# zhengjingsen/LidarDetection

Measured on AMD Instinct MI355X. Metric: frames/sec (fwd+NMS) PointPillar-KITTI, higher is better.
Workload: dtype f32; 1 GPU; PointPillar-KITTI bs=16 per GPU, fp32, eval BN folded: HIP voxelize + PFN; dense 2D backbone = first layer from the pillars (sparse implicit GEMM), stride-1 3x3 layers as Winograd F(4x4,3x3) on the fp32 MFMA, strided deblocks as one fused MFMA GEMM (all this repo's HIP), the two stride-2 3x3 layers MIOpen, stride-1 deblock + 1x1 heads hipBLASLt; exact HIP top-k + decode + batched rotated NMS; clou; replicas=1

## Files before the change

### include/lidar_hip.h

```cpp
#ifndef LIDAR_HIP_H
#define LIDAR_HIP_H

#include <stddef.h>
#include <stdint.h>

#ifdef __cplusplus
extern "C" {
#endif

#define LIDAR_OK 0
#define LIDAR_ERR_ARG (-1)
#define LIDAR_ERR_LAUNCH (-2)
#define LIDAR_ERR_WORKSPACE (-3)
#define LIDAR_ERR_UNSUPPORTED (-4)

size_t lidar_voxelize_workspace_bytes(int batch, int n_max, int max_voxels);
int lidar_voxelize_workspace_init(void *ws, size_t ws_bytes, int batch, int n_max, int max_voxels, void *stream);
int lidar_voxelize(const float *points, const int *point_offsets, int batch, int n_max, int num_features,
                   const float *range6, const float *voxel_size3, const int *grid3, int max_points,
                   int max_voxels, int compact, int algo, float *voxels, int *coords, int *num_points,
                   int *voxel_offsets, void *ws, size_t ws_bytes, void *stream);
int lidar_voxelize_hostoff(const float *points, const int *point_offsets, const int *host_offsets, int batch, int n_max,
                           int num_features, const float *range6, const float *voxel_size3, const int *grid3, int max_points,
                           int max_voxels, int compact, int algo, float *voxels, int *coords, int *num_points,
// ... 238 lines not shown
                            void *ws, size_t ws_bytes, void *stream);

size_t lidar_deconv_packed_floats(int K, int N);
int lidar_deconv_supported(int K, int s, int C_up);
int lidar_deconv_pack_weights(const float *W, int K, int N, float *packed, void *stream);
int lidar_deconv_gemm_nhwc(const float *in, int B, int h, int w, int K, const float *packed, const float *bias, int relu, int s, int C_up,
                           float *out, int out_C, int out_off, void *stream);

#define LIDAR_DECONV_TRAIN_MIN_K 16
#define LIDAR_DECONV_TRAIN_MIN_CUP 32
#define LIDAR_DECONV_TRAIN_MAX_C 512
int lidar_deconv_train_supported(int K, int s, int C_up);
size_t lidar_deconv_wgrad_workspace_bytes(int B, int h, int w, int K, int s, int C_up);
int lidar_deconv_dgrad_nhwc(const float *g, int g_ld, const float *W, int B, int h, int w, int K, int s, int C_up, float *dx, int dx_ld,
                            void *stream);
int lidar_deconv_wgrad_nhwc(const float *x, int x_ld, const float *g, int g_ld, int B, int h, int w, int K, int s, int C_up, float *dw,
                            void *ws, size_t ws_bytes, void *stream);

int lidar_anchor_scores(const float *head, long long n_loc, int row_stride, int cls_off, int anchors_per_loc, int num_class,
                        float score_thresh, float *scores, unsigned char *labels, void *stream);
int lidar_decode_topk(const float *head, int batch, long long locs_per_frame, int row_stride, int box_off, int dir_off,
                      int anchors_per_loc, int num_dir_bins, const long long *top_idx, int k, const float *anchors,
                      float dir_offset, float dir_limit_offset, float period, float *boxes, void *stream);
size_t lidar_topk_workspace_bytes(int batch, long long n);
int lidar_topk_workspace_init(void *ws, size_t ws_bytes, int batch, long long n, void *stream);
int lidar_anchor_scores_hist(const float *head, int batch, long long locs_per_frame, int row_stride, int cls_off, int anchors_per_loc,
                             int num_class, float score_thresh, float *scores, unsigned char *labels, void *ws, size_t ws_bytes,
                             void *stream);
int lidar_topk_desc(const float *scores, int batch, long long n, int k, float valid_min, float score_max, int hist_ready,
                    float *top_scores, long long *top_idx, int *counts, void *ws, size_t ws_bytes, void *stream);
int lidar_post_nms_gather(const float *boxes, const float *top_scores, const long long *top_idx, const unsigned char *labels,
                          const long long *keep, const int *num_keep, int batch, int k, long long n, int keep_stride, int post,
                          float *out_boxes, float *out_scores, long long *out_labels, int *out_num, void *stream);

size_t lidar_anchor_assign_workspace_bytes(int batch, int max_gt, int num_classes);
int lidar_anchor_assign(const float *const *anchors, const long long *counts, const long long *per_loc, const long long *out_off,
                        const float *matched, const float *unmatched, const int *remap, int num_classes, int anchor_dim,
                        long long a_total, const signed char *class_of_id, const float *gt, const float *gt_enlarged, int batch,
                        int max_gt, int gt_cols, int code_size, int sincos, int norm_by_num_examples, int *labels, float *targets,
                        float *weights, void *ws, size_t ws_bytes, void *stream);

int lidar_atss_assign_supported(const long long *counts, int num_sets, int anchor_dim, int gt_cols, int code_size, int sincos,
                                int topk, int max_gt, int match_height);
size_t lidar_atss_assign_workspace_bytes(int batch, int max_gt, int num_sets, int topk);
int lidar_atss_assign(const float *const *anchors, const long long *counts, int num_sets, int anchor_dim, const float *gt, int batch,
                      int max_gt, int gt_cols, int code_size, int sincos, int topk, int match_height, int *labels, float *targets,
// ... 126 lines not shown
```

### lidardetection_amd/_lib.py

```python
import ctypes as C
import os

_HERE = os.path.dirname(os.path.abspath(__file__))
SO_PATH = os.environ.get("LIDAR_HIP_SO") or os.path.join(_HERE, "csrc", "liblidar_hip.so")

vp, i32, f32, sz = C.c_void_p, C.c_int, C.c_float, C.c_size_t

SIGNATURES = {
    "lidar_voxelize_workspace_bytes": (sz, [i32, i32, i32]),
    "lidar_voxelize_workspace_init": (i32, [vp, sz, i32, i32, i32, vp]),
    "lidar_voxelize": (i32, [vp, vp, i32, i32, i32, vp, vp, vp, i32, i32, i32, i32, vp, vp, vp, vp, vp, sz, vp]),
    "lidar_voxelize_hostoff": (i32, [vp, vp, vp, i32, i32, i32, vp, vp, vp, i32, i32, i32, i32, vp, vp, vp, vp, vp, sz, vp]),
    "lidar_voxelize_error_flag": (i32, [vp, sz, i32, i32, i32]),
    "lidar_timer_create": (vp, []),
    "lidar_timer_destroy": (None, [vp]),
    "lidar_voxelize_time_next": (None, [vp]),
    "lidar_timer_elapsed_ms": (C.c_float, [vp]),
    "lidar_timer_parts_ms": (i32, [vp, vp]),
    "lidar_voxelize_set_error_mirror": (i32, [vp, sz, i32, i32, i32, vp, vp]),
    "lidar_pillar_vfe": (i32, [vp, vp, vp, i32, vp, i32, i32, vp, vp, vp, i32, vp, vp, i32, i32, i32, vp, vp]),
    "lidar_mean_vfe": (i32, [vp, vp, i32, i32, i32, i32, vp, vp]),
    "lidar_pillar_scatter_workspace_bytes": (sz, [i32, i32, i32]),
    "lidar_pillar_scatter": (i32, [vp, vp, i32, i32, vp, i32, i32, i32, i32, i32, vp, vp, sz, vp]),
    "lidar_pillar_scatter_update": (i32, [vp, vp, i32, i32, vp, i32, i32, i32, i32, vp, vp, vp, vp]),
# ... 97 lines not shown
    "lidar_wino43_pack_weights": (i32, [vp, i32, i32, vp, vp]),
    "lidar_wino43_conv3x3_nhwc": (i32, [vp, i32, i32, i32, i32, i32, vp, vp, i32, i32, vp, i32, i32, vp]),
    "lidar_wino43s_packed_floats": (sz, [i32, i32]),
    "lidar_wino43s_supported": (i32, [i32, i32]),
    "lidar_wino43s_pack_weights": (i32, [vp, i32, i32, vp, vp]),
    "lidar_wino43s_conv3x3_nhwc": (i32, [vp, i32, i32, i32, i32, i32, vp, vp, i32, i32, vp, i32, i32, vp]),
    "lidar_wino43_wgrad_supported": (i32, [i32, i32]),
    "lidar_wino43_wgrad_workspace_bytes": (sz, [i32, i32, i32, i32, i32]),
    "lidar_wino43_wgrad_nhwc": (i32, [vp, i32, vp, i32, i32, i32, i32, i32, i32, vp, vp, sz, vp]),
    "lidar_wino_conv3x3_grouped_nhwc": (i32, [vp, i32, i32, i32, i32, i32, i32, vp, vp, i32, vp, i32, i32, vp]),
    "lidar_wino_conv3x3_grouped_compact_nhwc": (i32, [vp, i32, i32, i32, i32, i32, i32, vp, vp, i32, vp, vp, vp, i32, i32, vp]),
    "lidar_deconv_packed_floats": (sz, [i32, i32]),
    "lidar_deconv_supported": (i32, [i32, i32, i32]),
    "lidar_deconv_pack_weights": (i32, [vp, i32, i32, vp, vp]),
    "lidar_deconv_gemm_nhwc": (i32, [vp, i32, i32, i32, i32, vp, vp, i32, i32, i32, vp, i32, i32, vp]),
    "lidar_deconv_train_supported": (i32, [i32, i32, i32]),
    "lidar_deconv_wgrad_workspace_bytes": (sz, [i32, i32, i32, i32, i32, i32]),
    "lidar_deconv_dgrad_nhwc": (i32, [vp, i32, vp, i32, i32, i32, i32, i32, i32, vp, i32, vp]),
    "lidar_deconv_wgrad_nhwc": (i32, [vp, i32, vp, i32, i32, i32, i32, i32, i32, i32, vp, vp, sz, vp]),
    "lidar_anchor_scores": (i32, [vp, C.c_longlong, i32, i32, i32, i32, f32, vp, vp, vp]),
    "lidar_decode_topk": (i32, [vp, i32, C.c_longlong, i32, i32, i32, i32, i32, vp, i32, vp, f32, f32, f32, vp, vp]),
    "lidar_topk_workspace_bytes": (sz, [i32, C.c_longlong]),
    "lidar_topk_workspace_init": (i32, [vp, sz, i32, C.c_longlong, vp]),
    "lidar_anchor_scores_hist": (i32, [vp, i32, C.c_longlong, i32, i32, i32, i32, f32, vp, vp, vp, sz, vp]),
    "lidar_topk_desc": (i32, [vp, i32, C.c_longlong, i32, f32, f32, i32, vp, vp, vp, vp, sz, vp]),
    "lidar_post_nms_gather": (i32, [vp, vp, vp, vp, vp, vp, i32, i32, C.c_longlong, i32, i32, vp, vp, vp, vp, vp]),
    "lidar_anchor_assign_workspace_bytes": (sz, [i32, i32, i32]),
    "lidar_anchor_assign": (i32, [vp, vp, vp, vp, vp, vp, vp, i32, i32, C.c_longlong, vp, vp, vp, i32, i32, i32, i32, i32, i32, vp,
                                  vp, vp, vp, sz, vp]),
    "lidar_atss_assign_supported": (i32, [vp, i32, i32, i32, i32, i32, i32, i32, i32]),
    "lidar_atss_assign_workspace_bytes": (sz, [i32, i32, i32, i32]),
    "lidar_atss_assign": (i32, [vp, vp, i32, i32, vp, i32, i32, i32, i32, i32, i32, i32, vp, vp, vp, vp, sz, vp]),
    "lidar_proposal_target_supported": (i32, [i32, i32, i32, i32]),
    "lidar_proposal_target": (i32, [vp, vp, vp, vp, vp, i32, i32, i32, i32, i32, i32, vp, i32, i32, f32, f32, f32, f32, f32, vp, vp,
                                    vp, vp, vp, vp, vp, vp, vp, vp, vp, vp, vp, vp, vp]),
    "lidar_augment_supported": (i32, [i32, i32, i32, i32]),
    "lidar_augment_workspace_bytes": (sz, [i32, i32, i32, i32]),
    "lidar_augment": (i32, [vp, vp, i32, i32, vp, vp, i32, i32, vp, vp, vp, vp, i32, i32, vp, i32, i32, vp, vp, vp, vp, vp, vp, vp,
                            vp, vp, vp, i32, i32, C.c_longlong, i32, vp, vp, vp, vp, vp, vp, sz, vp]),
    "lidar_anchor_loss_workspace_bytes": (sz, [i32, vp, i32]),
    "lidar_anchor_loss_forward": (i32, [vp, vp, vp, vp, vp, vp, i32, vp, vp, vp, i32, i32, C.c_longlong, i32, i32, i32, vp, vp, i32,
                                        vp, vp, sz, vp]),
    "lidar_anchor_loss_backward": (i32, [vp, vp, vp, vp, vp, vp, i32, vp, vp, vp, i32, i32, C.c_longlong, i32, i32, i32, vp, vp, i32,
                                         vp, vp, vp, vp, vp, sz, vp]),
    "lidar_roi_loss_supported": (i32, [i32, i32, i32, i32, i32, i32]),
    "lidar_roi_loss_workspace_bytes": (sz, [i32, i32]),
# ... 138 lines not shown
```

### lidardetection_amd/anchor_post.py

```python
import numpy as np
import torch

from . import _lib


_TOPK_WS = {}


def topk_supported(n, k, valid_min=None, hist=False):
    return n % 4 == 0 and 0 < k <= 4096 and n < 2 ** 31 and (not hist or valid_min is None or float(valid_min) > 0.0)


def drop_topk_workspace(ws):
    for key in [k for k, v in _TOPK_WS.items() if v is ws]:
        del _TOPK_WS[key]


def topk_workspace(batch, n, device):
    key = (str(device), int(batch), int(n), int(_lib.stream().value or 0))
    ws = _TOPK_WS.get(key)
    if ws is None:
        L = _lib.lib()
        nbytes = L.lidar_topk_workspace_bytes(batch, n)
        ws = torch.empty(nbytes, dtype=torch.uint8, device=device)
# ... 34 lines not shown
    _lib.check(_lib.lib().lidar_anchor_scores(_lib.ptr(head), n_loc, C, int(cls_off), int(anchors_per_loc), int(num_class),
                                              float(score_thresh), _lib.ptr(scores), _lib.ptr(labels), _lib.stream()),
               "lidar_anchor_scores")
    return scores, labels


def decode_topk(head, top_idx, anchors, anchors_per_loc, box_off, dir_off, num_dir_bins, dir_offset, dir_limit_offset):
    _lib.require_cuda(head, top_idx, anchors, allow=(torch.int64,))
    _lib.require_last(anchors, 7, "anchors")
    if top_idx.dtype != torch.int64:
        raise _lib.LidarHipError("decode_topk: top_idx must be int64 (torch.topk indices)")
    B, C = head.shape[0], head.shape[-1]
    locs = head.numel() // C // B
    k = top_idx.shape[1]
    boxes = torch.empty((B, k, 7), dtype=torch.float32, device=head.device)
    period = float(np.float32(2 * np.pi / num_dir_bins)) if num_dir_bins else 1.0
    _lib.check(_lib.lib().lidar_decode_topk(_lib.ptr(head), B, locs, C, int(box_off), int(dir_off), int(anchors_per_loc),
                                            int(num_dir_bins), _lib.ptr(top_idx), k, _lib.ptr(anchors), float(np.float32(dir_offset)),
                                            float(np.float32(dir_limit_offset)), period, _lib.ptr(boxes), _lib.stream()),
               "lidar_decode_topk")
    return boxes


def post_nms_gather(boxes, top_scores, top_idx, labels_all, keep, num_keep, post):
    _lib.require_cuda(boxes, top_scores, top_idx, labels_all, keep, num_keep, allow=(torch.int64, torch.uint8))
    if (boxes.dtype != torch.float32 or top_scores.dtype != torch.float32 or top_idx.dtype != torch.int64 or labels_all.dtype != torch.uint8
            or keep.dtype != torch.int64 or num_keep.dtype != torch.int32):
        raise _lib.LidarHipError("post_nms_gather: boxes / scores f32, top_idx / keep int64, labels uint8, num_keep int32")
    _lib.require_last(boxes, 7, "boxes")
    B, k = top_scores.shape
    n = labels_all.shape[1]
    post = int(post)
    dev = boxes.device
    out_boxes = torch.empty((B, post, 7), dtype=torch.float32, device=dev)
    out_scores = torch.empty((B, post), dtype=torch.float32, device=dev)
    out_labels = torch.empty((B, post), dtype=torch.int64, device=dev)
    out_num = torch.empty((B,), dtype=torch.int32, device=dev)
    _lib.check(_lib.lib().lidar_post_nms_gather(_lib.ptr(boxes), _lib.ptr(top_scores), _lib.ptr(top_idx), _lib.ptr(labels_all), _lib.ptr(keep),
                                                _lib.ptr(num_keep), B, k, n, keep.shape[1], post, _lib.ptr(out_boxes), _lib.ptr(out_scores),
                                                _lib.ptr(out_labels), _lib.ptr(out_num), _lib.stream()), "lidar_post_nms_gather")
    return out_boxes, out_scores, out_labels, out_num
```

### lidardetection_amd/bev_backbone.py

```python
import ctypes as C
import os
from typing import NamedTuple, Optional

import torch
import torch.nn as nn
import torch.nn.functional as F

from . import _lib, wino, workspace


def bias_act_(x, bias, relu=True, out=None, out_offset=0):
    _lib.require_cuda(bias)
    if not (x.is_cuda and x.dim() == 4 and x.is_contiguous(memory_format=torch.channels_last)):
        raise _lib.LidarHipError("bias_act_: expected a channels-last CUDA tensor")
    B, C, H, W = x.shape
    out, out_offset = (x, 0) if out is None else _lib.nhwc_out("bias_act_", B, (H, W), C, x.device, out, out_offset)
    _lib.check(_lib.lib().lidar_bias_act_nhwc(_lib.ptr(x), _lib.ptr(bias), B * H * W, C, int(bool(relu)), _lib.ptr(out),
                                              out.shape[1], int(out_offset), _lib.stream()), "lidar_bias_act_nhwc")
    return out


_LT_GEMM = [os.environ.get("LIDAR_BEV_LT_GEMM", "1") != "0"]
_SPLIT_MIN = [int(os.environ.get("LIDAR_BEV_SPLIT_MIN", "8"))]
_SPLIT = [int(os.environ.get("LIDAR_BEV_SPLIT", "2"))]
_WINO = [os.environ.get("LIDAR_BEV_WINO", "1") != "0"]
_DECONV = [os.environ.get("LIDAR_BEV_DECONV", "1") != "0"]
_SPARSE_FIRST = [os.environ.get("LIDAR_BEV_SPARSE_FIRST", "1") != "0"]


def _lt_gemm(a_ptr, M, K, w_kn, bias, relu, d_ptr, ldd, device):
    ws = workspace.get("dense_gemm", 32 << 20, device)
    st = _lib.lib().lidar_dense_gemm_bias_act(a_ptr, M, K, _lib.ptr(w_kn), w_kn.shape[1], _lib.ptr(bias), int(bool(relu)), d_ptr, ldd,
                                              _lib.ptr(ws), ws.numel(), _lib.stream())
    if st == -4:
        return False
    _lib.check(st, "lidar_dense_gemm_bias_act")
    return True


def _side_streams(device, n):
    from .spconv import conv as _sc, modules as _sm
    dev = torch.device(device)
    out = []
    for pool in (_sc._SIDE_STREAMS, _sm._RULEBOOK_STREAMS)[:n]:
        st = pool.get(dev)
        if st is None:
            st = pool[dev] = torch.cuda.Stream(dev, priority=-1)
        out.append(st)
    return out

# ... 181 lines not shown
                w, b = _fold(up.weight, bn, 1, up.bias)
                s = up.stride[0]
                if tuple(up.kernel_size) == tuple(up.stride) and s == up.stride[1] and \
                        tuple(up.padding) == (0, 0) and tuple(up.output_padding) == (0, 0):
                    w_kn = w.permute(0, 2, 3, 1).reshape(w.shape[0], -1).contiguous()
                    upc = FoldedDeblock("gemm", w_kn, None, b, s, ())
                    if _DECONV[0] and w.is_cuda and s > 1 and deconv_supported(w_kn.shape[0], s, b.numel()):
                        upc = upc._replace(kind="deconv_mfma", packed=deconv_pack(w_kn))
                else:
                    upc = FoldedDeblock("deconv", w.contiguous(memory_format=torch.channels_last), None, b, 0,
                                        (up.stride, up.padding, up.output_padding))
            else:
                w, b = _fold(up.weight, bn, 0, up.bias)
                upc = FoldedDeblock("conv", w.contiguous(memory_format=torch.channels_last), None, b, 0, (up.stride, up.padding))
            self.stages.append((convs, upc))
        self.up_channels = [up.shift.numel() for _, up in self.stages]
        for h in heads:
            assert tuple(h.kernel_size) == (1, 1) and tuple(h.stride) == (1, 1)
        self.head_split = [h.weight.shape[0] for h in heads]
        if heads:
            self.head_wt = torch.cat([h.weight.detach().flatten(1) for h in heads], 0).t().contiguous()
            self.head_b = torch.cat([h.bias.detach() if h.bias is not None else h.weight.new_zeros(h.weight.shape[0])
                                     for h in heads], 0).contiguous()
        self._cats = {}
        self._streams = None
        self._first_sparse = None
        c0 = self.stages[0][0][0]
        w0, b0, st0, pad0 = c0.weight, c0.shift, c0.stride, c0.pad
        k0 = w0.shape[2]
        if (w0.is_cuda and w0.shape[2] == w0.shape[3] and st0[0] == st0[1] and pad0[0] == pad0[1] and k0 * k0 <= 31
                and c0.dilation == (1, 1) and c0.groups == 1 and c0.zero_pad is None):
            from .spconv import ops as _sops
            if _sops.sorted_gemm_supported(k0 * k0, w0.shape[1], w0.shape[0]):
                self._first_sparse = (w0.permute(2, 3, 1, 0).reshape(k0 * k0, w0.shape[1], w0.shape[0]).contiguous(), b0, k0, int(st0[0]), int(pad0[0]))

    def first_layer_from_pillars(self, pm):
        from . import pillar_ops
        from .spconv import ops as _sops
        w9, b0, k0, st0, pad0 = self._first_sparse
        nbr, OH, OW = pillar_ops.pillar_conv_table(pm.coords, pm.B, pm.nx, pm.ny, k0, st0, pad0, pm.num_voxels_dev)
        order = _sops.mask_order(nbr)
        out = _sops.indice_conv_fused(pm.features, nbr, w9, b0, None, True, order)
        return out.view(pm.B, OH, OW, w9.shape[2]).permute(0, 3, 1, 2)

    def sparse_first_ok(self):
        return self._first_sparse is not None and _SPARSE_FIRST[0]

# ... 1 lines not shown
        x, cat, off = canvas, None, 0
        for si, (convs, up) in enumerate(self.stages):
            for ci, cv in enumerate(convs):
                if first_done and si == 0 and ci == 0:
                    continue
                if cv.wino is not None and _WINO[0] and x.is_contiguous(memory_format=torch.channels_last):
                    x = wino.conv3x3_auto(x, cv.wino, cv.weight.shape[0], cv.shift, True)
                    continue
                if cv.zero_pad is not None:
                    x = F.pad(x, cv.zero_pad)
                x = _cl(F.conv2d(x, cv.weight, None, cv.stride, cv.pad, cv.dilation, cv.groups))
                bias_act_(x, cv.shift)
            B, _, h, w = x.shape
            y = None
            if up.kind in ("deconv", "conv"):
                y = _cl((F.conv_transpose2d if up.kind == "deconv" else F.conv2d)(x, up.weight, None, *up.args))
            oh, ow = (h * up.stride, w * up.stride) if y is None else y.shape[2:]
            if cat is None:
                shape = (B, sum(self.up_channels), oh, ow)
                cat = self._cats.get(slot)
                if cat is None or cat.shape != shape or cat.device != x.device:
                    cat = self._cats[slot] = torch.empty(shape, dtype=torch.float32, device=x.device,
                                                         memory_format=torch.channels_last)
            if y is not None:
                bias_act_(y, up.shift, out=cat, out_offset=off)
            else:
                self._deblock_gemm(x, up, cat, off)
            off += up.shift.numel()
        return cat

    def _deblock_gemm(self, x, up, cat, off):
        B, K, h, w = x.shape
        if up.kind == "deconv_mfma" and deconv_fits(B, K, h, w, up.stride, cat.shape[1]):
            return deconv_gemm_into_(x, up.packed, up.shift, up.stride, cat, off)
        if up.kind == "gemm" and up.stride == 1 and _LT_GEMM[0]:
            if gemm_bias_act_into_(x, up.weight, up.shift, cat, off):
                return cat
            _LT_GEMM[0] = False
        y = rows_gemm(x.permute(0, 2, 3, 1).reshape(B * h * w, -1), up.weight)
        return bias_act_upsample_(y, up.shift, B, h, w, up.stride, cat, off)

    def stale(self):
        return params_key(self.sources) != self.source_key

    def merged(self, canvas):
        first_done = False
        if not torch.is_tensor(canvas):
            if self.sparse_first_ok():
                canvas, first_done = self.first_layer_from_pillars(canvas), True
            else:
                canvas = canvas.dense()
        B = canvas.shape[0]
        if 1 < _SPLIT[0] <= 2 and canvas.is_cuda and B % _SPLIT[0] == 0 and B // _SPLIT[0] >= _SPLIT_MIN[0]:
            return self._merged_split(canvas, _SPLIT[0], first_done)
        cat = self.features(canvas, first_done=first_done)
        B, C, H, W = cat.shape
        out = rows_gemm(cat.permute(0, 2, 3, 1).reshape(B * H * W, C), self.head_wt, self.head_b)
        return out.view(B, H, W, -1)

    def _merged_split(self, canvas, n, first_done=False):
        dev = canvas.device
        cur = torch.cuda.current_stream(dev)
        self._streams = _side_streams(dev, n)
        B, hb = canvas.shape[0], canvas.shape[0] // n
        out = None
        for i, st in enumerate(self._streams):
            st.wait_stream(cur)
            with torch.cuda.stream(st):
                cat = self.features(canvas[i * hb:(i + 1) * hb], slot=i + 1, first_done=first_done)
                _, C, H, W = cat.shape
                if out is None:
                    with torch.cuda.stream(cur):
                        out = torch.empty((B, H, W, self.head_wt.shape[1]), dtype=torch.float32, device=dev)
                    st.wait_stream(cur)
                out.record_stream(st)
                rows_gemm(cat.permute(0, 2, 3, 1).reshape(hb * H * W, C), self.head_wt, self.head_b, out=out[i * hb:(i + 1) * hb].view(hb * H * W, -1))
        for st in self._streams:
            cur.wait_stream(st)
        return out

    def __call__(self, canvas):
        return torch.split(self.merged(canvas), self.head_split, dim=-1)
```

### lidardetection_amd/csrc/anchor_post.hip

```cpp
#include "common.h"

__device__ __forceinline__ float sigmoid_ref(float x) { return 1.0f / (1.0f + expf(-x)); }

__global__ __launch_bounds__(256) void anchor_scores_kernel(const float *__restrict__ head, long long n_anchor, int row_stride,
                                                            int cls_off, int A, int ncls, float thresh,
                                                            float *__restrict__ scores, unsigned char *__restrict__ labels) {
    const long long i = (long long)blockIdx.x * 256 + threadIdx.x;
    if (i >= n_anchor) return;
    const long long loc = i / A;
    const int a = (int)(i - loc * A);
    const float *p = head + loc * row_stride + cls_off + a * ncls;
    float best = sigmoid_ref(p[0]);
    int bl = 0;
    for (int c = 1; c < ncls; ++c) {
        const float s = sigmoid_ref(p[c]);
        if (s > best) { best = s; bl = c; }
    }
    scores[i] = (best >= thresh) ? best : -1.0f;
    labels[i] = (unsigned char)bl;
}

__global__ __launch_bounds__(256) void decode_topk_kernel(const float *__restrict__ head, int batch, long long locs_per_frame,
                                                          int row_stride, int box_off, int dir_off, int A, int nbins,
                                                          const long long *__restrict__ top_idx, int k,
                                                          const float *__restrict__ anchors, float dir_offset,
                                                          float dir_limit_offset, float period, float *__restrict__ boxes) {
    const long long j = (long long)blockIdx.x * 256 + threadIdx.x;
    if (j >= (long long)batch * k) return;
    const int b = (int)(j / k);
    const long long idx = top_idx[j];
    const long long loc = idx / A;
    const int a = (int)(idx - loc * A);
    const float *row = head + ((long long)b * locs_per_frame + loc) * row_stride;
    const float *t = row + box_off + a * 7;
    const float *an = anchors + idx * 7;
    const float xa = an[0], ya = an[1], za = an[2], dxa = an[3], dya = an[4], dza = an[5], ra = an[6];
    const float diagonal = sqrtf(dxa * dxa + dya * dya);
    float *o = boxes + j * 7;
    o[0] = t[0] * diagonal + xa;
    o[1] = t[1] * diagonal + ya;
    o[2] = t[2] * dza + za;
    o[3] = expf(t[3]) * dxa;
    o[4] = expf(t[4]) * dya;
    o[5] = expf(t[5]) * dza;
    float rg = t[6] + ra;
    if (nbins > 0) {
        const float *d = row + dir_off + a * nbins;
        int lab = 0;
        float bestd = d[0];
        for (int c = 1; c < nbins; ++c)
            if (d[c] > bestd) { bestd = d[c]; lab = c; }
        const float inv_period = 1.0f / period;
        const float val = rg - dir_offset;
        const float fl = floorf(val * inv_period + dir_limit_offset);
        const float dir_rot = val - fl * period;
        rg = dir_rot + dir_offset + period * (float)lab;
    }
    o[6] = rg;
}

LIDAR_EXPORT int lidar_anchor_scores(const float *head, long long n_loc, int row_stride, int cls_off, int anchors_per_loc,
                                     int num_class, float score_thresh, float *scores, unsigned char *labels, void *stream) {
    if (n_loc < 0 || anchors_per_loc <= 0 || num_class <= 0 || cls_off < 0 ||
        cls_off + anchors_per_loc * num_class > row_stride)
        return LIDAR_ERR_ARG;
    if (n_loc == 0) return LIDAR_OK;
    if (!head || !scores || !labels) return LIDAR_ERR_ARG;
    const long long n = n_loc * anchors_per_loc;
    const long long blocks = (n + 255) / 256;
    if (blocks > 0x7fffffffll) return LIDAR_ERR_ARG;
    hipLaunchKernelGGL(anchor_scores_kernel, dim3((unsigned)blocks), dim3(256), 0, (hipStream_t)stream, head, n, row_stride, cls_off,
                       anchors_per_loc, num_class, score_thresh, scores, labels);
    return lidar_check_launch("lidar_anchor_scores");
}

LIDAR_EXPORT int lidar_decode_topk(const float *head, int batch, long long locs_per_frame, int row_stride, int box_off,
                                   int dir_off, int anchors_per_loc, int num_dir_bins, const long long *top_idx, int k,
                                   const float *anchors, float dir_offset, float dir_limit_offset, float period, float *boxes,
                                   void *stream) {
    if (batch < 0 || k < 0 || locs_per_frame < 0 || anchors_per_loc <= 0 || box_off < 0 ||
        box_off + anchors_per_loc * 7 > row_stride || num_dir_bins < 0 ||
        (num_dir_bins > 0 && (dir_off < 0 || dir_off + anchors_per_loc * num_dir_bins > row_stride)))
        return LIDAR_ERR_ARG;
    if (batch == 0 || k == 0) return LIDAR_OK;
    if (!head || !top_idx || !anchors || !boxes) return LIDAR_ERR_ARG;
    const long long n = (long long)batch * k;
    hipLaunchKernelGGL(decode_topk_kernel, dim3((unsigned)((n + 255) / 256)), dim3(256), 0, (hipStream_t)stream, head, batch,
                       locs_per_frame, row_stride, box_off, dir_off, anchors_per_loc, num_dir_bins, top_idx, k, anchors, dir_offset,
                       dir_limit_offset, period, boxes);
    return lidar_check_launch("lidar_decode_topk");
}

__global__ __launch_bounds__(256) void post_nms_gather_kernel(const float *__restrict__ boxes, const float *__restrict__ top_scores,
                                                              const long long *__restrict__ top_idx, const unsigned char *__restrict__ labels,
                                                              const long long *__restrict__ keep, const int *__restrict__ num_keep,
                                                              int batch, int k, long long n, int keep_stride, int post,
                                                              float *__restrict__ out_boxes, float *__restrict__ out_scores,
                                                              long long *__restrict__ out_labels, int *__restrict__ out_num) {
    const int j = blockIdx.x * 256 + threadIdx.x;
    if (j >= batch * post) return;
    const int b = j / post, s = j - b * post;
    const int nk = min(num_keep[b], post);
    if (s == 0) out_num[b] = nk;
    long long c = 0;
    if (s < nk) c = min(max(keep[(size_t)b * keep_stride + s], 0ll), (long long)k - 1);
    const float *src = boxes + ((size_t)b * k + c) * 7;
    float *dst = out_boxes + (size_t)j * 7;
#pragma unroll
    for (int q = 0; q < 7; ++q) dst[q] = src[q];
    out_scores[j] = top_scores[(size_t)b * k + c];
    const long long a = min(max(top_idx[(size_t)b * k + c], 0ll), n - 1);
    out_labels[j] = (long long)labels[(size_t)b * n + a] + 1;
}
// ... 14 lines not shown
```

### lidardetection_amd/pointpillar.py

```python
import numpy as np
import torch
import torch.nn as nn

from . import anchor_loss, anchor_post, pillar_ops, synth
from .bev_backbone import FoldedBEVBackbone, collect_params, params_key
from .bev_train import TrainBEVBackbone, _check_deblock, _check_wgrad
from .ext import iou3d_nms_cuda
from .voxelizer import BatchVoxelizer, grid_size_of

KITTI_ANCHORS = [
    ([3.9, 1.6, 1.56], [0, 1.57], -1.78),
    ([0.8, 0.6, 1.73], [0, 1.57], -0.6),
    ([1.76, 0.6, 1.73], [0, 1.57], -0.6),
]


def make_bev_backbone(cin=64, layer_nums=(3, 5, 5), strides=(2, 2, 2), filters=(64, 128, 256),
                      up_strides=(1, 2, 4), up_filters=(128, 128, 128)):
    blocks, deblocks = nn.ModuleList(), nn.ModuleList()
    c_in = [cin, *filters[:-1]]
    for i in range(len(layer_nums)):
        layers = [nn.ZeroPad2d(1), nn.Conv2d(c_in[i], filters[i], 3, stride=strides[i], padding=0, bias=False),
                  nn.BatchNorm2d(filters[i], eps=1e-3, momentum=0.01), nn.ReLU()]
        for _ in range(layer_nums[i]):
# ... 96 lines not shown
        if self._bev is None or self._bev.stale():
            self._bev = FoldedBEVBackbone(self.blocks, self.deblocks, [self.conv_cls, self.conv_box, self.conv_dir_cls])
        return self._bev

    def voxelize(self, points, point_offsets, host_offsets=None, timer=None):
        return self.voxelizer(points, point_offsets, self.n_max, compact=True, out=self._vox_out, resident=self.resident_voxels,
                              host_offsets=host_offsets, timer=timer)

    def vfe_scatter(self, vox):
        w, s, t = self._pfn_folded()
        total = vox["voxel_offsets"][self.B:self.B + 1]
        feat = pillar_ops.pillar_vfe(vox["voxels"], vox["voxel_num_points"], vox["voxel_coords"], w, s, t,
                                     self.voxel_size, self.pc_range, num_voxels_dev=total)
        if self.channels_last:
            def dense(f, c, n):
                if self._canvas is None:
                    self._canvas = pillar_ops.ResidentCanvas(self.B, f.shape[1], self.ny, self.nx, vox["voxels"].shape[0], f.device)
                return self._canvas.update(f, c, num_voxels_dev=n)
            if self.fold_bn and self._bev_folded().sparse_first_ok():
                return pillar_ops.PillarMap(feat, vox["voxel_coords"], total, self.B, self.nx, self.ny, dense)
            return dense(feat, vox["voxel_coords"], total)
        return pillar_ops.pillar_scatter(feat, vox["voxel_coords"], self.B, self.nx, self.ny, num_voxels_dev=total)

    def backbone_head(self, canvas):
        if self.fold_bn:
            return (self._bev_folded().merged(canvas),)
        return self.backbone_head_stock(canvas if torch.is_tensor(canvas) else canvas.dense())

    def split_heads(self, head):
        a = self.num_anchor_per_loc
        cls, box, dirs = torch.split(head, [a * self.num_class, a * 7, a * self.num_dir_bins], dim=-1)
        return (cls.reshape(self.B, -1, self.num_class), box.reshape(self.B, -1, 7), dirs.reshape(self.B, -1, self.num_dir_bins))

    def backbone_head_stock(self, canvas):
        ups, x = [], canvas
        for blk, de in zip(self.blocks, self.deblocks):
            x = blk(x)
            ups.append(de(x))
        return self._head_maps(torch.cat(ups, dim=1))

    def _head_maps(self, x):
        cls = self.conv_cls(x).permute(0, 2, 3, 1).reshape(self.B, -1, self.num_class)
        box = self.conv_box(x).permute(0, 2, 3, 1).reshape(self.B, -1, 7)
        dirs = self.conv_dir_cls(x).permute(0, 2, 3, 1).reshape(self.B, -1, self.num_dir_bins)
        return cls, box, dirs

    def backbone_head_train(self, canvas, wgrad="library", deblock="library"):
        _check_wgrad(wgrad, "PointPillarKITTI.backbone_head_train")
        _check_deblock(deblock, "PointPillarKITTI.backbone_head_train")
        if not self.channels_last:
            raise pillar_ops._lib.LidarHipError("PointPillarKITTI.backbone_head_train needs the channels-last model (channels_last=True)")
        key = ("_bev_train" if wgrad == "library" else "_bev_train_" + wgrad) + ("" if deblock == "library" else "_" + deblock)
        if self.__dict__.get(key) is None:
# ... 54 lines not shown
        diag = torch.sqrt(dxa ** 2 + dya ** 2)
        boxes = torch.cat([xt * diag + xa, yt * diag + ya, zt * dza + za, torch.exp(dxt) * dxa, torch.exp(dyt) * dya,
                           torch.exp(dzt) * dza, rt + ra], dim=-1)
        period = 2 * np.pi / self.num_dir_bins
        dir_labels = torch.max(dir_logits, dim=-1)[1]
        rot = limit_period(boxes[..., 6] - self.dir_offset, self.dir_limit_offset, period)
        boxes[..., 6] = rot + self.dir_offset + period * dir_labels.to(boxes.dtype)
        return boxes

    def post_process(self, *heads):
        if len(heads) == 1:
            return self.post_process_fused(heads[0])
        return self.post_process_torch(*heads)

    def select_topk(self, masked, k):
        if masked.is_cuda and anchor_post.topk_supported(masked.shape[1], k, self.score_thresh):
            return anchor_post.topk_desc(masked, k, self.score_thresh)[:2]
        return torch.topk(masked, k, dim=1)

    def post_process_fused(self, head):
        a = self.num_anchor_per_loc
        n = head.shape[1] * head.shape[2] * a if head.dim() == 4 else head.shape[1] * a
        k = min(self.nms_pre, n)
        if anchor_post.topk_supported(n, k, self.score_thresh, hist=True):
            ws = anchor_post.topk_workspace(head.shape[0], n, head.device)
            try:
                masked, labels_all = anchor_post.anchor_scores(head, a, self.num_class, self.score_thresh, cls_off=0, topk_ws=ws)
                top_scores, top_idx, counts = anchor_post.topk_desc(masked, k, self.score_thresh, ws, hist_ready=True)
            except BaseException:
                anchor_post.drop_topk_workspace(ws)
                raise
        else:
            masked, labels_all = anchor_post.anchor_scores(head, a, self.num_class, self.score_thresh, cls_off=0)
            top_scores, top_idx = torch.topk(masked, k, dim=1)
            counts = (top_scores >= self.score_thresh).sum(dim=1).to(torch.int32)
        boxes = anchor_post.decode_topk(head, top_idx, self.anchors, a, box_off=a * self.num_class,
                                        dir_off=a * (self.num_class + 7), num_dir_bins=self.num_dir_bins,
                                        dir_offset=self.dir_offset, dir_limit_offset=self.dir_limit_offset)
        post = min(self.nms_post, k)
        keep, num = iou3d_nms_cuda.nms_batch(boxes, counts, self.nms_thresh, max_keep=post)
        return anchor_post.post_nms_gather(boxes, top_scores, top_idx, labels_all, keep, num, post)

    def post_process_torch(self, cls, box, dirs):
        scores_all, labels_all = torch.sigmoid(cls).max(dim=-1)
        masked = torch.where(scores_all >= self.score_thresh, scores_all, scores_all.new_full((), -1.0))
        k = min(self.nms_pre, masked.shape[1])
        top_scores, top_idx = torch.topk(masked, k, dim=1)
        counts = (top_scores >= self.score_thresh).sum(dim=1).to(torch.int32)
        gi = top_idx.unsqueeze(-1)
        boxes = self.decode(torch.gather(box, 1, gi.expand(-1, -1, 7)), self.anchors[top_idx],
                            torch.gather(dirs, 1, gi.expand(-1, -1, self.num_dir_bins))).contiguous()
        return self._nms_and_gather(boxes, top_scores, top_idx, labels_all, counts, k)

    def _nms_and_gather(self, boxes, top_scores, top_idx, labels_all, counts, k):
        post = min(self.nms_post, k)
        keep, num = iou3d_nms_cuda.nms_batch(boxes, counts, self.nms_thresh, max_keep=post)
        sel = keep[:, :post].clamp_(0, k - 1)
        num = torch.clamp(num, max=post)
        valid = torch.arange(post, device=sel.device).unsqueeze(0) < num.unsqueeze(1)
        sel = torch.where(valid, sel, torch.zeros_like(sel))
        out_boxes = torch.gather(boxes, 1, sel.unsqueeze(-1).expand(-1, -1, 7))
# ... 10 lines not shown
```

Baseline: 3284 frames/s.

## Defer box/direction head GEMM to top-k rows only

The dense 1x1 head GEMM now computes only the class columns over every BEV location. The box and direction logits are computed later by a new HIP kernel, and only for the top-k selected anchors, reading the backbone concat buffers directly. A matching decode kernel consumes those compact rows. This cuts most of the head GEMM's FLOPs and output bandwidth. The cost is a gather-style per-row dot-product kernel, plus a staleness hazard if the concat buffers are overwritten before post-processing.

```diff
diff --git a/include/lidar_hip.h b/include/lidar_hip.h
--- a/include/lidar_hip.h
+++ b/include/lidar_hip.h
@@ -284,6 +284,13 @@
 int lidar_decode_topk(const float *head, int batch, long long locs_per_frame, int row_stride, int box_off, int dir_off,
                       int anchors_per_loc, int num_dir_bins, const long long *top_idx, int k, const float *anchors,
                       float dir_offset, float dir_limit_offset, float period, float *boxes, void *stream);
+#define LIDAR_HEAD_ROWS_MAX_C 1024
+int lidar_head_rows_supported(int C, int anchors_per_loc, int num_dir_bins, long long part_bytes);
+int lidar_head_rows(const float *part0, const float *part1, int n_parts, int frames_per_part, long long locs_per_frame, int C,
+                    const float *head_wt, int ldw, const float *head_b, int box_off, int dir_off, int anchors_per_loc, int num_dir_bins,
+                    const long long *idx, int batch, long long k, float *out, void *stream);
+int lidar_decode_topk_rows(const float *logits, int batch, int k, int num_dir_bins, const long long *top_idx, const float *anchors,
+                           float dir_offset, float dir_limit_offset, float period, float *boxes, void *stream);
 size_t lidar_topk_workspace_bytes(int batch, long long n);
 int lidar_topk_workspace_init(void *ws, size_t ws_bytes, int batch, long long n, void *stream);
 int lidar_anchor_scores_hist(const float *head, int batch, long long locs_per_frame, int row_stride, int cls_off, int anchors_per_loc,
diff --git a/lidardetection_amd/_lib.py b/lidardetection_amd/_lib.py
--- a/lidardetection_amd/_lib.py
+++ b/lidardetection_amd/_lib.py
@@ -143,6 +143,9 @@
     "lidar_decode_topk": (i32, [vp, i32, C.c_longlong, i32, i32, i32, i32, i32, vp, i32, vp, f32, f32, f32, vp, vp]),
     "lidar_topk_workspace_bytes": (sz, [i32, C.c_longlong]),
     "lidar_topk_workspace_init": (i32, [vp, sz, i32, C.c_longlong, vp]),
+    "lidar_head_rows_supported": (i32, [i32, i32, i32, C.c_longlong]),
+    "lidar_head_rows": (i32, [vp, vp, i32, i32, C.c_longlong, i32, vp, i32, vp, i32, i32, i32, i32, vp, i32, C.c_longlong, vp, vp]),
+    "lidar_decode_topk_rows": (i32, [vp, i32, i32, i32, vp, vp, f32, f32, f32, vp, vp]),
     "lidar_anchor_scores_hist": (i32, [vp, i32, C.c_longlong, i32, i32, i32, i32, f32, vp, vp, vp, sz, vp]),
     "lidar_topk_desc": (i32, [vp, i32, C.c_longlong, i32, f32, f32, i32, vp, vp, vp, vp, sz, vp]),
     "lidar_post_nms_gather": (i32, [vp, vp, vp, vp, vp, vp, i32, i32, C.c_longlong, i32, i32, vp, vp, vp, vp, vp]),
diff --git a/lidardetection_amd/anchor_post.py b/lidardetection_amd/anchor_post.py
--- a/lidardetection_amd/anchor_post.py
+++ b/lidardetection_amd/anchor_post.py
@@ -80,6 +80,54 @@
     return boxes
 
 
+def head_rows_supported(C, anchors_per_loc, num_dir_bins, part_bytes=0):
+    return bool(_lib.lib().lidar_head_rows_supported(int(C), int(anchors_per_loc), int(num_dir_bins), int(part_bytes)))
+
+
+def head_rows(parts, head_wt, head_b, anchors_per_loc, box_off, dir_off, num_dir_bins, top_idx=None, batch=None):
+    parts = list(parts)
+    _lib.require_cuda(*parts, head_wt, head_b)
+    if not 1 <= len(parts) <= 2 or any(p.shape != parts[0].shape or not p.is_contiguous() for p in parts):
+        raise _lib.LidarHipError("head_rows: one or two contiguous NHWC part maps of one shape")
+    fpp, C = parts[0].shape[0], parts[0].shape[-1]
+    locs = parts[0].numel() // max(fpp * C, 1)
+    B = fpp * len(parts) if batch is None else int(batch)
+    nc = 7 + int(num_dir_bins)
+    if not head_wt.is_contiguous() or head_wt.dim() != 2 or head_wt.shape[0] != C or head_b.numel() != head_wt.shape[1]:
+        raise _lib.LidarHipError("head_rows: head_wt must be a contiguous (C, N) matrix and head_b its (N,) bias")
+    if not head_rows_supported(C, anchors_per_loc, num_dir_bins, parts[0].numel() * 4):
+        raise _lib.LidarHipError(f"head_rows: unsupported shape (C {C}, A {anchors_per_loc}, bins {num_dir_bins}, "
+                                 f"{parts[0].numel() * 4} bytes per part)")
+    if top_idx is None:
+        k, idx_ptr = locs * int(anchors_per_loc), None
+    else:
+        _lib.require_cuda(top_idx, allow=(torch.int64,))
+        if top_idx.dtype != torch.int64 or top_idx.dim() != 2 or top_idx.shape[0] != B or not top_idx.is_contiguous():
+            raise _lib.LidarHipError("head_rows: top_idx must be a contiguous int64 (B, k) tensor")
+        k, idx_ptr = top_idx.shape[1], _lib.ptr(top_idx)
+    out = torch.empty((B, k, nc), dtype=torch.float32, device=parts[0].device)
+    _lib.check(_lib.lib().lidar_head_rows(_lib.ptr(parts[0]), _lib.ptr(parts[-1]), len(parts), fpp, locs, C, _lib.ptr(head_wt),
+                                          head_wt.shape[1], _lib.ptr(head_b), int(box_off), int(dir_off), int(anchors_per_loc),
+                                          int(num_dir_bins), idx_ptr, B, k, _lib.ptr(out), _lib.stream()), "lidar_head_rows")
+    return out
+
+
+def decode_topk_rows(logits, top_idx, anchors, num_dir_bins, dir_offset, dir_limit_offset):
+    _lib.require_cuda(logits, top_idx, anchors, allow=(torch.int64,))
+    _lib.require_last(anchors, 7, "anchors")
+    B, k = top_idx.shape
+    if top_idx.dtype != torch.int64 or not top_idx.is_contiguous():
+        raise _lib.LidarHipError("decode_topk_rows: top_idx must be contiguous int64 (B, k)")
+    if logits.dtype != torch.float32 or not logits.is_contiguous() or tuple(logits.shape) != (B, k, 7 + int(num_dir_bins)):
+        raise _lib.LidarHipError("decode_topk_rows: logits must be contiguous float32 (B, k, 7 + num_dir_bins)")
+    boxes = torch.empty((B, k, 7), dtype=torch.float32, device=logits.device)
+    period = float(np.float32(2 * np.pi / num_dir_bins)) if num_dir_bins else 1.0
+    _lib.check(_lib.lib().lidar_decode_topk_rows(_lib.ptr(logits), B, k, int(num_dir_bins), _lib.ptr(top_idx), _lib.ptr(anchors),
+                                                 float(np.float32(dir_offset)), float(np.float32(dir_limit_offset)), period,
+                                                 _lib.ptr(boxes), _lib.stream()), "lidar_decode_topk_rows")
+    return boxes
+
+
 def post_nms_gather(boxes, top_scores, top_idx, labels_all, keep, num_keep, post):
     _lib.require_cuda(boxes, top_scores, top_idx, labels_all, keep, num_keep, allow=(torch.int64, torch.uint8))
     if (boxes.dtype != torch.float32 or top_scores.dtype != torch.float32 or top_idx.dtype != torch.int64 or labels_all.dtype != torch.uint8
diff --git a/lidardetection_amd/bev_backbone.py b/lidardetection_amd/bev_backbone.py
--- a/lidardetection_amd/bev_backbone.py
+++ b/lidardetection_amd/bev_backbone.py
@@ -26,6 +26,29 @@
 _WINO = [os.environ.get("LIDAR_BEV_WINO", "1") != "0"]
 _DECONV = [os.environ.get("LIDAR_BEV_DECONV", "1") != "0"]
 _SPARSE_FIRST = [os.environ.get("LIDAR_BEV_SPARSE_FIRST", "1") != "0"]
+_HEAD_DEFER = [os.environ.get("LIDAR_HEAD_DEFER", "1") != "0"]
+
+
+class DeferredHead:
+
+    def __init__(self, owner, slots, parts, head_wt, head_b, box_off, dir_off):
+        self.owner, self.slots, self.parts = owner, tuple(slots), tuple(parts)
+        self.gens = tuple(owner._cat_gen[s] for s in slots)
+        self.head_wt, self.head_b, self.box_off, self.dir_off = head_wt, head_b, int(box_off), int(dir_off)
+        self.frames_per_part = parts[0].shape[0]
+
+    def stale(self):
+        o = self.owner
+        return any(o._cat_gen.get(s) != g or o._cats.get(s) is not p for s, g, p in zip(self.slots, self.gens, self.parts))
+
+    def rows(self, anchors_per_loc, num_dir_bins, top_idx=None, who="DeferredHead.rows"):
+        from . import anchor_post
+        if self.stale():
+            raise _lib.LidarHipError(f"{who}: this deferred head is stale — the backbone's concat buffers it reads its box / direction "
+                                     "columns from were overwritten by a later forward (post-process a head before the next "
+                                     "backbone_head call, or run with LIDAR_HEAD_DEFER=0)")
+        return anchor_post.head_rows([p.permute(0, 2, 3, 1) for p in self.parts], self.head_wt, self.head_b, anchors_per_loc,
+                                     self.box_off, self.dir_off, num_dir_bins, top_idx)
 
 
 def _lt_gemm(a_ptr, M, K, w_kn, bias, relu, d_ptr, ldd, device):
@@ -253,7 +276,10 @@
             self.head_wt = torch.cat([h.weight.detach().flatten(1) for h in heads], 0).t().contiguous()
             self.head_b = torch.cat([h.bias.detach() if h.bias is not None else h.weight.new_zeros(h.weight.shape[0])
                                      for h in heads], 0).contiguous()
+            self.head0_wt = self.head_wt[:, :self.head_split[0]].contiguous()
+            self.head0_b = self.head_b[:self.head_split[0]].contiguous()
         self._cats = {}
+        self._cat_gen = {}
         self._streams = None
         self._first_sparse = None
         c0 = self.stages[0][0][0]
@@ -301,6 +327,7 @@
                 if cat is None or cat.shape != shape or cat.device != x.device:
                     cat = self._cats[slot] = torch.empty(shape, dtype=torch.float32, device=x.device,
                                                          memory_format=torch.channels_last)
+                self._cat_gen[slot] = self._cat_gen.get(slot, 0) + 1
             if y is not None:
                 bias_act_(y, up.shift, out=cat, out_offset=off)
             else:
@@ -322,7 +349,12 @@
     def stale(self):
         return params_key(self.sources) != self.source_key
 
-    def merged(self, canvas):
+    def _defer_ok(self, cat_bytes):
+        from . import anchor_post
+        return (_HEAD_DEFER[0] and len(self.head_split) > 1 and self.head_wt.is_cuda
+                and anchor_post.head_rows_supported(self.head_wt.shape[0], 1, 0, cat_bytes))
+
+    def merged(self, canvas, defer=False):
         first_done = False
         if not torch.is_tensor(canvas):
             if self.sparse_first_ok():
@@ -331,31 +363,41 @@
                 canvas = canvas.dense()
         B = canvas.shape[0]
         if 1 < _SPLIT[0] <= 2 and canvas.is_cuda and B % _SPLIT[0] == 0 and B // _SPLIT[0] >= _SPLIT_MIN[0]:
-            return self._merged_split(canvas, _SPLIT[0], first_done)
+            return self._merged_split(canvas, _SPLIT[0], first_done, defer)
         cat = self.features(canvas, first_done=first_done)
         B, C, H, W = cat.shape
-        out = rows_gemm(cat.permute(0, 2, 3, 1).reshape(B * H * W, C), self.head_wt, self.head_b)
-        return out.view(B, H, W, -1)
-
-    def _merged_split(self, canvas, n, first_done=False):
+        defer = bool(defer) and self._defer_ok(cat.numel() * 4)
+        wt, b = (self.head0_wt, self.head0_b) if defer else (self.head_wt, self.head_b)
+        out = rows_gemm(cat.permute(0, 2, 3, 1).reshape(B * H * W, C), wt, b).view(B, H, W, -1)
+        if defer:
+            out.deferred = DeferredHead(self, (0,), (cat,), self.head_wt, self.head_b, self.head_split[0], sum(self.head_split[:2]))
+        return out
+
+    def _merged_split(self, canvas, n, first_done=False, defer=False):
         dev = canvas.device
         cur = torch.cuda.current_stream(dev)
         self._streams = _side_streams(dev, n)
         B, hb = canvas.shape[0], canvas.shape[0] // n
-        out = None
+        out, cats, wt, b = None, [], self.head_wt, self.head_b
         for i, st in enumerate(self._streams):
             st.wait_stream(cur)
             with torch.cuda.stream(st):
                 cat = self.features(canvas[i * hb:(i + 1) * hb], slot=i + 1, first_done=first_done)
+                cats.append(cat)
                 _, C, H, W = cat.shape
                 if out is None:
+                    defer = bool(defer) and self._defer_ok(cat.numel() * 4)
+                    if defer:
+                        wt, b = self.head0_wt, self.head0_b
                     with torch.cuda.stream(cur):
-                        out = torch.empty((B, H, W, self.head_wt.shape[1]), dtype=torch.float32, device=dev)
+                        out = torch.empty((B, H, W, wt.shape[1]), dtype=torch.float32, device=dev)
                     st.wait_stream(cur)
                 out.record_stream(st)
-                rows_gemm(cat.permute(0, 2, 3, 1).reshape(hb * H * W, C), self.head_wt, self.head_b, out=out[i * hb:(i + 1) * hb].view(hb * H * W, -1))
+                rows_gemm(cat.permute(0, 2, 3, 1).reshape(hb * H * W, C), wt, b, out=out[i * hb:(i + 1) * hb].view(hb * H * W, -1))
         for st in self._streams:
             cur.wait_stream(st)
+        if defer:
+            out.deferred = DeferredHead(self, range(1, n + 1), cats, self.head_wt, self.head_b, self.head_split[0], sum(self.head_split[:2]))
         return out
 
     def __call__(self, canvas):
diff --git a/lidardetection_amd/csrc/anchor_post.hip b/lidardetection_amd/csrc/anchor_post.hip
--- a/lidardetection_amd/csrc/anchor_post.hip
+++ b/lidardetection_amd/csrc/anchor_post.hip
@@ -20,6 +20,31 @@
     labels[i] = (unsigned char)bl;
 }
 
+__device__ __forceinline__ void decode_box(const float *__restrict__ t, const float *__restrict__ d, int nbins, const float *__restrict__ an,
+                                           float dir_offset, float dir_limit_offset, float period, float *__restrict__ o) {
+    const float xa = an[0], ya = an[1], za = an[2], dxa = an[3], dya = an[4], dza = an[5], ra = an[6];
+    const float diagonal = sqrtf(dxa * dxa + dya * dya);
+    o[0] = t[0] * diagonal + xa;
+    o[1] = t[1] * diagonal + ya;
+    o[2] = t[2] * dza + za;
+    o[3] = expf(t[3]) * dxa;
+    o[4] = expf(t[4]) * dya;
+    o[5] = expf(t[5]) * dza;
+    float rg = t[6] + ra;
+    if (nbins > 0) {
+        int lab = 0;
+        float bestd = d[0];
+        for (int c = 1; c < nbins; ++c)
+            if (d[c] > bestd) { bestd = d[c]; lab = c; }
+        const float inv_period = 1.0f / period;
+        const float val = rg - dir_offset;
+        const float fl = floorf(val * inv_period + dir_limit_offset);
+        const float dir_rot = val - fl * period;
+        rg = dir_rot + dir_offset + period * (float)lab;
+    }
+    o[6] = rg;
+}
+
 __global__ __launch_bounds__(256) void decode_topk_kernel(const float *__restrict__ head, int batch, long long locs_per_frame,
                                                           int row_stride, int box_off, int dir_off, int A, int nbins,
                                                           const long long *__restrict__ top_idx, int k,
@@ -32,31 +57,18 @@
     const long long loc = idx / A;
     const int a = (int)(idx - loc * A);
     const float *row = head + ((long long)b * locs_per_frame + loc) * row_stride;
-    const float *t = row + box_off + a * 7;
-    const float *an = anchors + idx * 7;
-    const float xa = an[0], ya = an[1], za = an[2], dxa = an[3], dya = an[4], dza = an[5], ra = an[6];
-    const float diagonal = sqrtf(dxa * dxa + dya * dya);
-    float *o = boxes + j * 7;
-    o[0] = t[0] * diagonal + xa;
-    o[1] = t[1] * diagonal + ya;
-    o[2] = t[2] * dza + za;
-    o[3] = expf(t[3]) * dxa;
-    o[4] = expf(t[4]) * dya;
-    o[5] = expf(t[5]) * dza;
-    float rg = t[6] + ra;
-    if (nbins > 0) {
-        const float *d = row + dir_off + a * nbins;
-        int lab = 0;
-        float bestd = d[0];
-        for (int c = 1; c < nbins; ++c)
-            if (d[c] > bestd) { bestd = d[c]; lab = c; }
-        const float inv_period = 1.0f / period;
-        const float val = rg - dir_offset;
-        const float fl = floorf(val * inv_period + dir_limit_offset);
-        const float dir_rot = val - fl * period;
-        rg = dir_rot + dir_offset + period * (float)lab;
-    }
-    o[6] = rg;
+    decode_box(row + box_off + a * 7, row + dir_off + a * nbins, nbins, anchors + idx * 7, dir_offset, dir_limit_offset, period,
+               boxes + j * 7);
+}
+
+__global__ __launch_bounds__(256) void decode_topk_rows_kernel(const float *__restrict__ logits, long long n, int nbins,
+                                                               const long long *__restrict__ top_idx, const float *__restrict__ anchors,
+                                                               float dir_offset, float dir_limit_offset, float period,
+                                                               float *__restrict__ boxes) {
+    const long long j = (long long)blockIdx.x * 256 + threadIdx.x;
+    if (j >= n) return;
+    const float *t = logits + j * (7 + nbins);
+    decode_box(t, t + 7, nbins, anchors + top_idx[j] * 7, dir_offset, dir_limit_offset, period, boxes + j * 7);
 }
 
 LIDAR_EXPORT int lidar_anchor_scores(const float *head, long long n_loc, int row_stride, int cls_off, int anchors_per_loc,
@@ -89,6 +101,20 @@
                        locs_per_frame, row_stride, box_off, dir_off, anchors_per_loc, num_dir_bins, top_idx, k, anchors, dir_offset,
                        dir_limit_offset, period, boxes);
     return lidar_check_launch("lidar_decode_topk");
+}
+
+LIDAR_EXPORT int lidar_decode_topk_rows(const float *logits, int batch, int k, int num_dir_bins, const long long *top_idx,
+                                        const float *anchors, float dir_offset, float dir_limit_offset, float period, float *boxes,
+                                        void *stream) {
+    if (batch < 0 || k < 0 || num_dir_bins < 0) return LIDAR_ERR_ARG;
+    if (batch == 0 || k == 0) return LIDAR_OK;
+    if (!logits || !top_idx || !anchors || !boxes) return LIDAR_ERR_ARG;
+    const long long n = (long long)batch * k;
+    const long long blocks = (n + 255) / 256;
+    if (blocks > 0x7fffffffll) return LIDAR_ERR_ARG;
+    hipLaunchKernelGGL(decode_topk_rows_kernel, dim3((unsigned)blocks), dim3(256), 0, (hipStream_t)stream, logits, n, num_dir_bins, top_idx,
+                       anchors, dir_offset, dir_limit_offset, period, boxes);
+    return lidar_check_launch("lidar_decode_topk_rows");
 }
 
 __global__ __launch_bounds__(256) void post_nms_gather_kernel(const float *__restrict__ boxes, const float *__restrict__ top_scores,
diff --git a/lidardetection_amd/csrc/head_rows.hip b/lidardetection_amd/csrc/head_rows.hip
--- /dev/null
+++ b/lidardetection_amd/csrc/head_rows.hip
@@ -0,0 +1,171 @@
+#include "common.h"
+
+#define HR_THREADS 1024
+#define HR_WAVES (HR_THREADS / 64)
+#define HR_MAX_C 1024
+#define HR_MAX_A 8
+#define HR_MAX_BINS 4
+#define HR_LDS_MAX (128 * 1024)
+
+struct HrArgs {
+    const float *part[2];
+    const float *wt, *bias;
+    const long long *list;
+    float *out;
+    long long locs, k, total;
+    int frames_per_part, C, ldw, box_off, dir_off, A;
+};
+
+template <int NB>
+__device__ __forceinline__ int hr_col(const HrArgs &p, int a, int q) {
+    return q < 7 ? p.box_off + a * 7 + q : p.dir_off + a * NB + (q - 7);
+}
+
+__device__ __forceinline__ const float4 *hr_row(const HrArgs &p, long long j, int &a) {
+    const long long f = j / p.k;
+    long long idx = p.list ? p.list[j] : j - f * p.k;
+    idx = min(max(idx, 0ll), p.locs * p.A - 1);
+    const long long loc = idx / p.A;
+    a = (int)(idx - loc * p.A);
+    const int part = (int)(f / p.frames_per_part);
+    const long long lf = f - (long long)part * p.frames_per_part;
+    return reinterpret_cast<const float4 *>(p.part[part] + (lf * p.locs + loc) * p.C);
+}
+
+template <int NB, bool LDSW>
+__device__ __forceinline__ void hr_group(const HrArgs &p, const float *s_w, int pitch, int a, int g, const float4 x, float (&acc)[7 + NB]) {
+    constexpr int NC = 7 + NB;
+#pragma unroll
+    for (int q = 0; q < NC; ++q) {
+        float4 w;
+        if (LDSW) {
+            w = *reinterpret_cast<const float4 *>(s_w + (size_t)(a * NC + q) * pitch + 4 * g);
+        } else {
+            const float *c = p.wt + (size_t)(4 * g) * p.ldw + hr_col<NB>(p, a, q);
+            w = make_float4(c[0], c[p.ldw], c[2 * (size_t)p.ldw], c[3 * (size_t)p.ldw]);
+        }
+        acc[q] = fmaf(x.x, w.x, acc[q]);
+        acc[q] = fmaf(x.y, w.y, acc[q]);
+        acc[q] = fmaf(x.z, w.z, acc[q]);
+        acc[q] = fmaf(x.w, w.w, acc[q]);
+    }
+}
+
+template <int NB, bool LDSW>
+__global__ __launch_bounds__(HR_THREADS) void head_rows_kernel(const HrArgs p) {
+    constexpr int NC = 7 + NB;
+    extern __shared__ float4 s_hr4[];
+    float *s_w = reinterpret_cast<float *>(s_hr4);
+    const int pitch = p.C + 4;
+    if (LDSW) {
+        const int ncol = p.A * NC;
+        for (int e = threadIdx.x; e < p.C * ncol; e += HR_THREADS) {
+            const int i = e / ncol, cl = e - i * ncol;
+            const int a = cl / NC, q = cl - a * NC;
+            s_w[(size_t)cl * pitch + i] = p.wt[(size_t)i * p.ldw + hr_col<NB>(p, a, q)];
+        }
+        __syncthreads();
+    }
+    const int lane = lane_id(), c4 = p.C >> 2;
+    const long long nw = (long long)gridDim.x * HR_WAVES;
+    long long j = (long long)blockIdx.x * HR_WAVES + (threadIdx.x >> 6);
+    if (j >= p.total) return;
+    const float4 zero4 = make_float4(0.f, 0.f, 0.f, 0.f);
+    int a = 0;
+    const float4 *row = hr_row(p, j, a);
+    float4 x0 = lane < c4 ? row[lane] : zero4, x1 = lane + 64 < c4 ? row[lane + 64] : zero4;
+    while (true) {
+        const long long jn = j + nw;
+        int an = 0;
+        const float4 *rown = row;
+        float4 n0 = zero4, n1 = zero4;
+        if (jn < p.total) {
+            rown = hr_row(p, jn, an);
+            if (lane < c4) n0 = rown[lane];
+            if (lane + 64 < c4) n1 = rown[lane + 64];
+        }
+        float acc[NC];
+#pragma unroll
+        for (int q = 0; q < NC; ++q) acc[q] = 0.0f;
+        if (lane < c4) hr_group<NB, LDSW>(p, s_w, pitch, a, lane, x0, acc);
+        if (lane + 64 < c4) hr_group<NB, LDSW>(p, s_w, pitch, a, lane + 64, x1, acc);
+        for (int g = lane + 128; g < c4; g += 64) hr_group<NB, LDSW>(p, s_w, pitch, a, g, row[g], acc);
+        float mine = 0.0f;
+        int col = 0;
+#pragma unroll
+        for (int q = 0; q < NC; ++q) {
+            const float s = wave_sum(acc[q]);
+            if (lane == q) { mine = s; col = hr_col<NB>(p, a, q); }
+        }
+        if (lane < NC) p.out[j * NC + lane] = mine + p.bias[col];
+        if (jn >= p.total) break;
+        j = jn; a = an; row = rown; x0 = n0; x1 = n1;
+    }
+}
+
+static int hr_cu_count() {
+    static int cus[64] = {};
+    int dev = 0, n = 0;
+    if (hipGetDevice(&dev) != hipSuccess) return 256;
+    dev &= 63;
+    if (cus[dev] == 0) cus[dev] = (hipDeviceGetAttribute(&n, hipDeviceAttributeMultiprocessorCount, dev) == hipSuccess && n > 0) ? n : 256;
+    return cus[dev];
+}
+
+template <int NB>
+static int hr_launch(const HrArgs &p, hipStream_t stream) {
+    const size_t lds = (size_t)p.A * (7 + NB) * (p.C + 4) * sizeof(float);
+    long long blocks = (p.total + HR_WAVES - 1) / HR_WAVES;
+    const long long cap = (long long)hr_cu_count() * (lds <= HR_LDS_MAX ? 1 : 2);
+    if (blocks > cap) blocks = cap;
+    if (lds <= HR_LDS_MAX) {
+        static bool attr_set[64] = {};
+        int dev_id = 0;
+        (void)hipGetDevice(&dev_id);
+        dev_id &= 63;
+        if (!attr_set[dev_id]) {
+            (void)hipFuncSetAttribute(reinterpret_cast<const void *>(&head_rows_kernel<NB, true>), hipFuncAttributeMaxDynamicSharedMemorySize,
+                                      HR_LDS_MAX);
+            attr_set[dev_id] = true;
+        }
+        hipLaunchKernelGGL((head_rows_kernel<NB, true>), dim3((unsigned)blocks), dim3(HR_THREADS), lds, stream, p);
+    } else {
+        hipLaunchKernelGGL((head_rows_kernel<NB, false>), dim3((unsigned)blocks), dim3(HR_THREADS), 0, stream, p);
+    }
+    return lidar_check_launch("lidar_head_rows");
+}
+
+LIDAR_EXPORT int lidar_head_rows_supported(int C, int anchors_per_loc, int num_dir_bins, long long part_bytes) {
+    return C >= 4 && C <= HR_MAX_C && (C & 3) == 0 && anchors_per_loc >= 1 && anchors_per_loc <= HR_MAX_A && num_dir_bins >= 0 &&
+           num_dir_bins <= HR_MAX_BINS && part_bytes >= 0 && part_bytes < 0x7fffffffll;
+}
+
+LIDAR_EXPORT int lidar_head_rows(const float *part0, const float *part1, int n_parts, int frames_per_part, long long locs_per_frame, int C,
+                                 const float *head_wt, int ldw, const float *head_b, int box_off, int dir_off, int anchors_per_loc,
+                                 int num_dir_bins, const long long *idx, int batch, long long k, float *out, void *stream) {
+    if (batch < 0 || k < 0 || locs_per_frame < 0 || frames_per_part <= 0 || n_parts < 1 || n_parts > 2 || ldw <= 0 || box_off < 0 ||
+        dir_off < 0 || locs_per_frame > 0x7fffffffll / 4 ||
+        !lidar_head_rows_supported(C, anchors_per_loc, num_dir_bins, (long long)frames_per_part * locs_per_frame * (C > 0 ? C : 1) * 4))
+        return LIDAR_ERR_ARG;
+    if (box_off + anchors_per_loc * 7 > ldw || (num_dir_bins > 0 && dir_off + anchors_per_loc * num_dir_bins > ldw) ||
+        (long long)n_parts * frames_per_part < batch)
+        return LIDAR_ERR_ARG;
+    if (!idx && k != locs_per_frame * anchors_per_loc) return LIDAR_ERR_ARG;
+    if (batch == 0 || k == 0) return LIDAR_OK;
+    if (locs_per_frame == 0) return LIDAR_ERR_ARG;
+    if (!part0 || (n_parts == 2 && !part1) || !head_wt || !head_b || !out) return LIDAR_ERR_ARG;
+    if ((reinterpret_cast<uintptr_t>(part0) & 15) || (reinterpret_cast<uintptr_t>(part1) & 15)) return LIDAR_ERR_ARG;
+    if ((long long)batch * k > 0x7fffffffll * 16) return LIDAR_ERR_ARG;
+    HrArgs p;
+    p.part[0] = part0; p.part[1] = n_parts == 2 ? part1 : part0;
+    p.wt = head_wt; p.bias = head_b; p.list = idx; p.out = out;
+    p.locs = locs_per_frame; p.k = k; p.total = (long long)batch * k;
+    p.frames_per_part = frames_per_part; p.C = C; p.ldw = ldw; p.box_off = box_off; p.dir_off = dir_off; p.A = anchors_per_loc;
+    switch (num_dir_bins) {
+    case 0: return hr_launch<0>(p, (hipStream_t)stream);
+    case 1: return hr_launch<1>(p, (hipStream_t)stream);
+    case 2: return hr_launch<2>(p, (hipStream_t)stream);
+    case 3: return hr_launch<3>(p, (hipStream_t)stream);
+    default: return hr_launch<4>(p, (hipStream_t)stream);
+    }
+}
diff --git a/lidardetection_amd/pointpillar.py b/lidardetection_amd/pointpillar.py
--- a/lidardetection_amd/pointpillar.py
+++ b/lidardetection_amd/pointpillar.py
@@ -142,13 +142,19 @@
             return dense(feat, vox["voxel_coords"], total)
         return pillar_ops.pillar_scatter(feat, vox["voxel_coords"], self.B, self.nx, self.ny, num_voxels_dev=total)
 
-    def backbone_head(self, canvas):
+    def backbone_head(self, canvas, defer=None):
         if self.fold_bn:
-            return (self._bev_folded().merged(canvas),)
+            if defer is None:
+                defer = anchor_post.head_rows_supported(self.conv_cls.in_channels, self.num_anchor_per_loc, self.num_dir_bins)
+            return (self._bev_folded().merged(canvas, defer=bool(defer)),)
         return self.backbone_head_stock(canvas if torch.is_tensor(canvas) else canvas.dense())
 
     def split_heads(self, head):
         a = self.num_anchor_per_loc
+        rec = getattr(head, "deferred", None)
+        if rec is not None:
+            logits = rec.rows(a, self.num_dir_bins, None, "split_heads")
+            return head.reshape(self.B, -1, self.num_class), logits[..., :7], logits[..., 7:]
         cls, box, dirs = torch.split(head, [a * self.num_class, a * 7, a * self.num_dir_bins], dim=-1)
         return (cls.reshape(self.B, -1, self.num_class), box.reshape(self.B, -1, 7), dirs.reshape(self.B, -1, self.num_dir_bins))
 
@@ -249,6 +255,9 @@
         a = self.num_anchor_per_loc
         n = head.shape[1] * head.shape[2] * a if head.dim() == 4 else head.shape[1] * a
         k = min(self.nms_pre, n)
+        rec = getattr(head, "deferred", None)
+        if rec is not None and rec.stale():
+            rec.rows(a, self.num_dir_bins, None, "post_process")
         if anchor_post.topk_supported(n, k, self.score_thresh, hist=True):
             ws = anchor_post.topk_workspace(head.shape[0], n, head.device)
             try:
@@ -261,9 +270,13 @@
             masked, labels_all = anchor_post.anchor_scores(head, a, self.num_class, self.score_thresh, cls_off=0)
             top_scores, top_idx = torch.topk(masked, k, dim=1)
             counts = (top_scores >= self.score_thresh).sum(dim=1).to(torch.int32)
-        boxes = anchor_post.decode_topk(head, top_idx, self.anchors, a, box_off=a * self.num_class,
-                                        dir_off=a * (self.num_class + 7), num_dir_bins=self.num_dir_bins,
-                                        dir_offset=self.dir_offset, dir_limit_offset=self.dir_limit_offset)
+        if rec is not None:
+            logits = rec.rows(a, self.num_dir_bins, top_idx.contiguous(), "post_process")
+            boxes = anchor_post.decode_topk_rows(logits, top_idx, self.anchors, self.num_dir_bins, self.dir_offset, self.dir_limit_offset)
+        else:
+            boxes = anchor_post.decode_topk(head, top_idx, self.anchors, a, box_off=a * self.num_class,
+                                            dir_off=a * (self.num_class + 7), num_dir_bins=self.num_dir_bins,
+                                            dir_offset=self.dir_offset, dir_limit_offset=self.dir_limit_offset)
         post = min(self.nms_post, k)
         keep, num = iou3d_nms_cuda.nms_batch(boxes, counts, self.nms_thresh, max_keep=post)
         return anchor_post.post_nms_gather(boxes, top_scores, top_idx, labels_all, keep, num, post)
```

Result: faster. 3358 frames/s (median of 6 runs) (+2.3%).
